# ADicksonLab/AGDIFF

Hardware: AMD Instinct MI355X
Metric: conformers/sec (whole node), GEOM-Drugs 5000-step sampling (higher is better)
Workload: dtype f16x3

## Files before the change

agdiff_amd/csrc/api.hip:

```cpp
#include "common.hpp"
#include <algorithm>
#include <mutex>
#include <vector>

extern "C" int agdiff_abi_version(void) { return AGDIFF_ABI_VERSION; }

extern "C" int agdiff_conv_chunk_tiles(int64_t max_edges) {
  const int64_t tiles = (max_edges + AG_TW - 1) / AG_TW;
  int c = 1;
  while (c < AGDIFF_MAX_CHUNK_TILES && tiles / (2 * c) >= 16 * 2048) c *= 2;
  return c;
}

extern "C" int agdiff_group_order(const int32_t* need, int32_t n, int32_t k, int32_t gt, int32_t* order_out) {
  if (n < 0 || k < 0 || (gt != 1 && gt != 2 && gt != 4) || (n > 0 && (!need || !order_out))) return AGDIFF_ERR_ARG;
  if (n == 0) return AGDIFF_OK;
  auto row = [&](int i) { return need + (size_t)i * k; };
  std::vector<int> total(n, 0);
  for (int i = 0; i < n; ++i)
    for (int t = 0; t < k; ++t) total[i] += row(i)[t];
  auto start_order = [&](int r, std::vector<int>& o) {
    o.resize(n);
    for (int i = 0; i < n; ++i) o[i] = i;
    std::stable_sort(o.begin(), o.end(), [&](int a, int b) {
// ... 157 lines not shown
  }
  return f;
}

int local_branch(const agdiff_params_t* p, const agdiff_topo_t* topo, const agdiff_ws_t* ws, const float* pos, int flags,
                 bool rows_from_global, hipEvent_t rows_ready, void* stream, bool split = false,
                 hipEvent_t split_ready = nullptr) {
  const int64_t ltiles = (topo->num_local + AG_TW - 1) / AG_TW;
  const int64_t ctiles = (topo->num_local_canon + AG_TW - 1) / AG_TW;
  const bool canon = !(flags & AGDIFF_FWD_GRAPH_GIVEN) && topo->num_local_canon > 0;
  const bool front_did_local = (flags & AGDIFF_FWD_GRAPH_READY) != 0;
  if (!(flags & AGDIFF_FWD_GRAPH_GIVEN) && !front_did_local) AG_TRY(agdiff_local_lengths(topo, ws, pos, stream));
  if (rows_from_global) {
    if (hipStreamWaitEvent((hipStream_t)stream, rows_ready, 0) != hipSuccess) return AGDIFF_ERR_LAUNCH;
  } else if (topo->num_local > 0) {
    if (canon && split) {
      const int lp = agdiff_local_poly_enabled(p, topo, ws);
      if (lp != 0 && !front_did_local) AG_TRY(agdiff_edge_scales_split(p, topo, ws, 2, stream));
      if (lp == 1) {
        AG_TRY(agdiff_local_edge_rows(p, topo, ws, stream));
      } else {
        AG_TRY(agdiff_edge_encoder(p, ws->num_local_canon, ctiles, ws->lc_len, topo->lc_type, ws->l_attr_frag, ws->l_attr_rows,
                                   topo->lp_row, topo->lc_ppos, topo->lc_pmir, stream));
        AG_TRY(agdiff_edge_scales_split(p, topo, ws, 1, stream));
      }
    } else if (canon)
      AG_TRY(agdiff_local_edge_rows(p, topo, ws, stream));
    else
      AG_TRY(agdiff_edge_encoder(p, ws->num_local, ltiles, ws->l_len, topo->loc_type, nullptr, ws->l_attr_rows, nullptr,
                                 nullptr, nullptr, stream));
  }
  if (split && split_ready && hipEventRecord(split_ready, (hipStream_t)stream) != hipSuccess) return AGDIFF_ERR_LAUNCH;
  AG_TRY(agdiff_gin_encoder(p, topo, ws, canon ? 1 : 0, stream));
  if (topo->num_local > 0) {
    agdiff_head_params_t hl = p->head_local;
    hl.range_rows = ws->range_rows;
    if (canon)
      AG_TRY(agdiff_pair_head(&hl, ws->num_local_canon, ctiles, topo->lc_src, topo->lc_dst, ws->hl, nullptr,
                              ws->l_attr_rows, topo->lc_pos, topo->lc_mir, ws->l_inv, stream));
    else
      AG_TRY(agdiff_pair_head(&hl, ws->num_local, ltiles, topo->loc_src, topo->loc_dst, ws->hl, nullptr,
                              ws->l_attr_rows, nullptr, nullptr, ws->l_inv, stream));
  }
  return AGDIFF_OK;
}

int global_front(const agdiff_params_t* p, const agdiff_topo_t* topo, const agdiff_ws_t* ws, const float* pos, int flags,
                 bool rows_for_local, void* stream) {
  const int64_t etiles = (topo->max_edges + AG_TW - 1) / AG_TW;
  if (!(flags & AGDIFF_FWD_GRAPH_GIVEN))
    AG_TRY(agdiff_graph_build(topo, ws, pos, (flags & AGDIFF_FWD_NO_RADIUS) ? 0.0f : p->cutoff, stream));
  AG_TRY(agdiff_edge_scales(p, topo, ws, (flags & AGDIFF_FWD_GRAPH_GIVEN) ? 0 : 1, stream));
  if (flags & AGDIFF_FWD_GRAPH_GIVEN) {
    AG_TRY(agdiff_edge_encoder(p, ws->num_edges, etiles, ws->e_len, ws->e_type, ws->e_attr, nullptr, nullptr, nullptr,
                               nullptr, stream));
  } else {
    AG_TRY(agdiff_edge_encoder(p, ws->num_canon, etiles, ws->c_len, ws->c_type, ws->e_attr,
                               rows_for_local ? ws->l_attr_rows : nullptr, rows_for_local ? ws->e_loc : nullptr, ws->c_pos,
                               ws->c_mir, stream));
  }
  return AGDIFF_OK;
}

int global_back(const agdiff_params_t* p, const agdiff_topo_t* topo, const agdiff_ws_t* ws, int flags, void* stream) {
  const int64_t etiles = (topo->max_edges + AG_TW - 1) / AG_TW;
  for (int k = 0; k <= p->num_convs; ++k) {
    AG_TRY(agdiff_schnet_node_stage(p, topo, ws, k, stream));
    if (k < p->num_convs) {
      ProfScope prof(stream);
      AG_TRY(agdiff_cfconv_fused(p, topo, ws, k, stream));
    }
  }
  agdiff_head_params_t hg = p->head_global;
  hg.range_rows = ws->range_rows;
  if (flags & AGDIFF_FWD_GRAPH_GIVEN) {
    AG_TRY(agdiff_pair_head(&hg, ws->num_edges, etiles, ws->e_src, ws->e_dst, ws->h, ws->e_attr, nullptr,
// ... 164 lines not shown
```

agdiff_amd/csrc/edge.hip:

```cpp
#include "common.hpp"

namespace {

__device__ __forceinline__ const lds_u32x4* ag_lds_base(const lds_u32x4* p, int lane) {
  const lds_u32x4* b = p + lane;
  asm volatile("" : "+v"(b));
  return b;
}

struct EncArgs {
  const float* fe_w;
  const float* fe_b;
  const float* t1;
  const float* w1_pk;
  const float* t3;
  const float* w23_pk;
  const float* w4_pk;
  const float* b4;
  const int32_t* n_dev;
  const float* e_len;
  const int32_t* e_type;
  float* out_frag;
  float* out_rows;
  const int32_t* row_index;
// ... 787 lines not shown
        ag_load_slice_pieces(r[0], r[1], hs, k, lane);
        ag_load_slice_pieces(r[2], r[3], ht, k, lane);
      };
      auto finish = [&](AgIn<MODE>& dst, const f32x4 (&r)[4]) {
        ag_cvt(ag_permute4(r[0] * r[2], to_op), ag_permute4(r[1] * r[3], to_op), dst);
      };
      fetch(raw, 0);
      finish(sl[0], raw);
      const lds_u32x4* lw1_l = ag_lds_base(lw1, lane);
#pragma unroll
      for (int k = 0; k < 4; ++k) {
        if (k + 1 < 4) fetch(raw, k + 1);
        if (k & 1) ag_dense_lds<MODE, false, true, 1, 8, 1, 0>(sl, y1, lw1_l + (k * 8) * 128, 0);
        else ag_dense_lds<MODE, false, true, 1, 8, 0, 0>(sl, y1, lw1_l + (k * 8) * 128, 0);
        if (k + 1 < 4) finish(sl[(k + 1) & 1], raw);
      }
      AgIn<MODE> ph[NKT];
      ag_poly_features<MODE, NKT>(d, a.two_over_rc, q, ph);
      ag_dense_lds<MODE, false, true, NKT, 8, 0, 0>(ph, y1, ag_lds_base(lwp, lane), 0);
    }
    ag_head_act<8>(y1, a.hp.act);
    f32x4 y2[4];
    ag_init_vec<4>(y2, a.hp.b2, q);
    {
      AgIn<MODE> y1b[4];
      ag_report_range<MODE>(ag_absmax<MODE, 8>(y1, 0.0f), a.hp.range_rows, s, valid);
      ag_cvt_tiles<MODE, 4, 0>(y1, y1b);
      ag_dense_lds<MODE, false, false, 4, 4, 0, 0>(y1b, y2, ag_lds_base(lw2, lane), 0);
    }
    ag_head_act<4>(y2, a.hp.act);
    const float o = ag_dot_vec<4>(y2, a.hp.w3, q) + a.hp.b3;
    if (valid && q == 0) {
      a.out[pe] = o;
      if (pm >= 0) a.out[pm] = o;
    }
  }
}

template <int F>
__global__ void __launch_bounds__(AG_WG) k_cfconv_aggregate(const float* __restrict__ x, const float* __restrict__ W,
                                                            const int32_t* __restrict__ in_ptr,
                                                            const int32_t* __restrict__ src, int64_t n,
                                                            float* __restrict__ out) {
  constexpr int LPE = F / 4;
  constexpr int EPI = 64 / LPE;
  const int lane = ag_lane();
  const int64_t node = (int64_t)blockIdx.x * 4 + ag_wave_in_wg();
  if (node >= n) return;
  const int lo = in_ptr[node], hi = in_ptr[node + 1];
  const int sub = lane / LPE, fl = (lane % LPE) * 4;
  f32x4 acc = {0.f, 0.f, 0.f, 0.f};
  for (int e = lo + sub; e < hi; e += EPI) {
    const f32x4 w = ag_ld4(W + (size_t)e * F + fl);
    const f32x4 xv = ag_ld4(x + (size_t)src[e] * F + fl);
    acc += w * xv;
  }
#pragma unroll
  for (int o = LPE; o < 64; o <<= 1) {
#pragma unroll
    for (int q = 0; q < 4; ++q) acc[q] += __shfl_xor(acc[q], o);
  }
  if (sub == 0) ag_st4(out + (size_t)node * F + fl, acc);
}

}

// ... 300 lines not shown

extern "C" int agdiff_pair_head(const agdiff_head_params_t* hp, const int32_t* n_edges_dev, int64_t max_tiles,
                                const int32_t* src, const int32_t* dst, const float* node_h, const float* attr_frag,
                                const float* attr_rows, const int32_t* pos_index, const int32_t* mir_index, float* out,
                                void* stream) {
  if (!hp || !n_edges_dev || !src || !dst || !node_h || (!attr_frag == !attr_rows) || !out || max_tiles < 0 ||
      (!pos_index != !mir_index))
    return AGDIFF_ERR_ARG;
  if (max_tiles == 0) return AGDIFF_OK;
  HeadArgs a;
  a.hp = *hp;
  a.n_dev = n_edges_dev;
  a.src = src;
  a.dst = dst;
  a.node_h = node_h;
  a.attr_frag = attr_frag;
  a.attr_rows = attr_rows;
  a.pos_index = pos_index;
  a.mir_index = mir_index;
  a.out = out;
  a.max_tiles = max_tiles;
  int64_t wgs = (max_tiles + AG_PERSIST_WAVES - 1) / AG_PERSIST_WAVES;
  if (wgs > 256) wgs = 256;
  const size_t smem = (size_t)80 * 2048;
  static std::atomic<uint64_t> attr_done{0};
  if (!ag_allow_big_lds(attr_done, smem, k_pair_head<AG_BF3>, k_pair_head<AG_F32>, k_pair_head<AG_H3>)) return AGDIFF_ERR_LAUNCH;
  ag_by_mode(hp->precision, [&](auto M) {
    k_pair_head<decltype(M)::value><<<dim3((unsigned)wgs), dim3(64 * AG_PERSIST_WAVES), smem, (hipStream_t)stream>>>(a);
  });
  AG_CHECK_LAUNCH();
  return AGDIFF_OK;
}

extern "C" int agdiff_cfconv_aggregate(const float* x, const float* W, const int32_t* in_ptr, const int32_t* src,
                                       int64_t num_nodes, int32_t F, float* out, void* stream) {
  if (!x || !W || !in_ptr || !src || !out || num_nodes < 0) return AGDIFF_ERR_ARG;
  if (F != 64 && F != 128) return AGDIFF_ERR_LIMIT;
  if (num_nodes == 0) return AGDIFF_OK;
  dim3 grid((unsigned)((num_nodes + 3) / 4));
  if (F == 128)
    k_cfconv_aggregate<128><<<grid, dim3(AG_WG), 0, (hipStream_t)stream>>>(x, W, in_ptr, src, num_nodes, out);
  else
    k_cfconv_aggregate<64><<<grid, dim3(AG_WG), 0, (hipStream_t)stream>>>(x, W, in_ptr, src, num_nodes, out);
  AG_CHECK_LAUNCH();
  return AGDIFF_OK;
}
```

agdiff_amd/packing.py:

```python
import ctypes

import numpy as np

from . import _lib

H = 128


def _np(sd, key):
    return sd[key].detach().cpu().double().numpy()


def bf16_round(x32):
    u = np.ascontiguousarray(x32, dtype=np.float32).view(np.uint32).astype(np.uint64)
    r = ((u + 0x7FFF + ((u >> 16) & 1)) >> 16).astype(np.uint32)
    return r.astype(np.uint16), (r << 16).astype(np.uint32).view(np.float32)


def _block_columns():
    lane = np.arange(64)
    j = np.arange(8)
    return 16 * (j >> 2)[None, :] + 4 * (lane >> 4)[:, None] + (j & 3)[None, :]


# ... 112 lines not shown
    G.append(2 * T8 * T8 - 1)
    G.append(2 * G[2] * T8 - T8)
    G.append(2 * G[2] * G[2] - 1)
    G.append(2 * G[4] * T8 - G[3])
    G.append(2 * G[3] * G[3] - 1)
    G.append(2 * G[6] * T8 - G[5])
    while len(G) < K // 8:
        G.append(2 * T8 * G[-1] - G[-2])
    return np.stack([G[f // 8] * T[f % 8] for f in range(K)], axis=-1)


def fit_poly(fn, cutoff, K, lo=0.0):
    k = np.arange(K)
    xn = np.cos(np.pi * (k + 0.5) / K)
    half = (cutoff - lo) / 2.0
    fv = fn(lo + (xn + 1.0) * half)
    b = np.polynomial.chebyshev.chebfit(xn, fv, K - 1)
    c = np.linalg.solve(poly_basis_matrix(K), b)
    dg = np.linspace(lo, cutoff, 4097)
    ref = fn(dg)
    err = np.abs(poly_features((dg - lo) / half - 1.0, K) @ c - ref).max() / max(np.abs(ref).max(), 1e-300)
    return c.T, float(err)


ATTR_FAR_FACTOR = 10.0
ATTR_POLY_MAX_SETS = 9


def fit_attr_far(sd, cfg, typ):
    key = (_poly_weights_digest(sd, cfg), float(cfg.cutoff), int(typ), "attr_far")
    if key not in _FIT_CACHE:
        fn = _edge_attr_fn(sd, "edge_encoder_global", typ)
        c, err = fit_poly(lambda d: fn(d).numpy(), ATTR_FAR_FACTOR * float(cfg.cutoff), 32, lo=float(cfg.cutoff))
        _FIT_CACHE[key] = (c[:, poly_feature_order(1)], err)
    return _FIT_CACHE[key]


def _edge_attr_fn(sd, e, typ):
    import torch
    import torch.nn.functional as F
    g = lambda k: sd[e + k].detach().cpu().double()
    few, feb = g(".feature_expansion.weight"), g(".feature_expansion.bias")
    W0, b0, W2, b2 = g(".edge_feature_mlp.0.weight"), g(".edge_feature_mlp.0.bias"), g(".edge_feature_mlp.2.weight"), g(".edge_feature_mlp.2.bias")
    C0, c0, C2, c2 = g(".combination_mlp.0.weight"), g(".combination_mlp.0.bias"), g(".combination_mlp.2.weight"), g(".combination_mlp.2.bias")
    emb = g(".bond_emb.weight")[int(typ)]

    def fn(d):
        d = torch.from_numpy(np.ascontiguousarray(d, dtype=np.float64)).view(-1, 1)
        x = F.gelu(F.linear(d, few, feb))
        b = emb.expand(d.shape[0], -1)
        h = F.linear(F.gelu(F.linear(torch.cat([x, b], 1), W0, b0)), W2, b2)
        return F.linear(F.gelu(F.linear(torch.cat([h, b], 1), C0, c0)), C2, c2)
    return fn


def encoder_activation_by_type(sd, cfg, far=10.0):
    import torch
    import torch.nn.functional as F
    e = "edge_encoder_global"
    g = lambda k: sd[k].detach().cpu().double()
    few, feb = g(e + ".feature_expansion.weight"), g(e + ".feature_expansion.bias")
    W0, b0, W2, b2 = g(e + ".edge_feature_mlp.0.weight"), g(e + ".edge_feature_mlp.0.bias"), g(e + ".edge_feature_mlp.2.weight"), g(e + ".edge_feature_mlp.2.bias")
    C0, c0, C2, c2 = g(e + ".combination_mlp.0.weight"), g(e + ".combination_mlp.0.bias"), g(e + ".combination_mlp.2.weight"), g(e + ".combination_mlp.2.bias")
    emb = g(e + ".bond_emb.weight")
    d = torch.linspace(0.0, float(far) * float(cfg.cutoff), 1025, dtype=torch.float64).view(-1, 1)
    x = F.gelu(F.linear(d, few, feb))
# ... 531 lines not shown
            self.poly_errors["type%d" % t] = err
            if err > POLY_TOL or len(self.local_slots) >= max_slots or not self._type_fits_plan(t, mats, err):
                self.poly_refused_types.add(t)
                continue
            self.local_slots[t] = len(self.local_slots)
            self._typed_mats[t] = mats
            added = True
        if not added:
            return not any(int(t) in self.poly_refused_types for t in types)
        by_slot = sorted(self.local_slots, key=self.local_slots.get)
        self._pack_filter_sets()
        if kt == 1:
            sets = [pack_blocks(self._typed_mats[t]["edge_attr_poly_pk"], mode=self._mode_local) for t in by_slot]
            far_table = np.full(100, -1, dtype=np.int32)
            room = max(0, ATTR_POLY_MAX_SETS - len(by_slot)) if self.attr_far else 0
            prio = {24: 0, 23: 1, 1: 2}
            for t in sorted(by_slot, key=lambda ty: (prio.get(ty, 3), ty)):
                if room <= 0:
                    break
                c, err = fit_attr_far(self._sd, self._cfg, t)
                self.poly_errors["type%d_far" % t] = err
                if err > POLY_TOL:
                    continue
                far_table[t] = len(sets)
                sets.append(pack_blocks(c, mode=self._mode_local))
                room -= 1
            attr_sets = np.concatenate(sets)
            self.typed_attr_flat = torch.from_numpy(attr_sets).to(self.device)
            prm.attr_poly_typed_pk = ctypes.c_void_p(self.typed_attr_flat.data_ptr())
            self.attr_far_table = torch.from_numpy(far_table).to(self.device)
            prm.attr_poly_far_set = ctypes.c_void_p(self.attr_far_table.data_ptr())
            prm.attr_poly_far_slots = int((far_table >= 0).sum())
            prm.attr_poly_far_hi = ATTR_FAR_FACTOR * float(self._cfg.cutoff)
        table = np.full(100, -1, dtype=np.int32)
        for t, sl in self.local_slots.items():
            table[t] = sl
        self.slot_table = torch.from_numpy(table).to(self.device)
        prm.poly_type_slot = ctypes.c_void_p(self.slot_table.data_ptr())
        prm.poly_num_slots = len(by_slot)
        sm = [0, 0]
        for t in self.local_slots:
            sm[t >> 6] |= 1 << (t & 63)
        for w in (0, 1):
            prm.poly_slot_mask[w] = sm[w] - (1 << 64) if sm[w] >= (1 << 63) else sm[w]
        return not any(int(t) in self.poly_refused_types for t in types)

    TUNING = ("share_rows_min_nodes", "node_ldsw_min_tiles", "node_split_max_tiles", "serial_branches", "local_poly_off",
              "attr_poly_off", "poly_lds_sets", "cfconv_four_min_quads", "cfconv_quad_tiles")

    def set_tuning(self, **kw):
        for k, v in kw.items():
            if k not in self.TUNING:
                raise KeyError("unknown tuning field %r (known: %s)" % (k, ", ".join(self.TUNING)))
            setattr(self.struct, "tune_" + k, int(v))

    def view(self, name):
        o = self.offsets[name]
        return self.flat[o:o + self.sizes[name]]

    def update_schnet_embedding(self, weight):
        self.view("schnet_emb").copy_(weight.detach().reshape(-1).to(self.flat.dtype))
```

agdiff_amd/topology.py:

```python
import numpy as np

from . import _lib
from .synth import extend_graph_order_np


def _to_np(x):
    if hasattr(x, "detach"):
        x = x.detach().cpu().numpy()
    return np.asarray(x)


def batch_fingerprint(atom_type, bond_index, bond_type, batch, num_graphs, extend_order):
    def wsum(cols, mults):
        if hasattr(cols[0], "detach"):
            import torch
            n = int(cols[0].reshape(-1).shape[0])
            if n == 0:
                return 0
            acc = torch.zeros(n, dtype=torch.int64, device=cols[0].device)
            for c, m in zip(cols, mults):
                acc += c.reshape(-1).to(torch.int64) * m
            acc = (acc + 12345) * torch.arange(1, n + 1, dtype=torch.int64, device=acc.device)
            return int(acc.sum().item())
        cols = [np.asarray(c).reshape(-1).astype(np.int64) for c in cols]
# ... 33 lines not shown

def extend_graph_order_sparse(n, bond_src, bond_dst, bond_type, order=3, num_types=None):
    from .synth import NUM_BOND_TYPES
    num_types = NUM_BOND_TYPES if num_types is None else num_types
    n = int(n)
    bs, bd = np.asarray(bond_src, dtype=np.int64), np.asarray(bond_dst, dtype=np.int64)
    bkey, inv = np.unique(bs * n + bd, return_inverse=True)
    tsum = np.zeros(bkey.shape[0], dtype=np.int64)
    np.add.at(tsum, inv.reshape(-1), np.asarray(bond_type, dtype=np.int64))
    offdiag = (bkey // n) != (bkey % n)
    adj = bkey[offdiag]
    a_src, a_dst = adj // n, adj % n
    nb_ptr = np.concatenate([[0], np.cumsum(np.bincount(a_src, minlength=n))])
    seen = np.union1d(np.arange(n, dtype=np.int64) * (n + 1), adj)
    frontier = adj
    keys, types = [bkey], [tsum]
    for k in range(2, order + 1):
        f_src, f_dst = frontier // n, frontier % n
        deg = nb_ptr[f_dst + 1] - nb_ptr[f_dst]
        rep_src = np.repeat(f_src, deg)
        first = np.repeat(nb_ptr[f_dst], deg)
        within = np.arange(rep_src.shape[0]) - np.repeat(np.cumsum(deg) - deg, deg)
        cand = np.unique(rep_src * n + a_dst[first + within])
        frontier = np.setdiff1d(cand, seen, assume_unique=True)
        seen = np.union1d(seen, frontier)
        keys.append(frontier)
        types.append(np.full(frontier.shape[0], num_types + k - 1, dtype=np.int64))
    key = np.concatenate(keys)
    typ = np.concatenate(types)
    o = np.argsort(key, kind="stable")
    key, typ = key[o], typ[o]
    keep = typ != 0
    return key[keep] // n, key[keep] % n, typ[keep]


class BatchTopology:
    GROUP_MIN_NODES = ((6144, 4), (3072, 2))

    def __init__(self, atom_type, bond_index, bond_type, batch, num_graphs=None, extend_order=False,
                 order=3, device="cuda", group_targets=None, radius_column=True):
        import torch
        at = _to_np(atom_type).astype(np.int64)
        bi = _to_np(bond_index).astype(np.int64).reshape(2, -1)
        bt = _to_np(bond_type).astype(np.int64).reshape(-1)
        ba = _to_np(batch).astype(np.int64)
        self.fingerprint = batch_fingerprint(at, bi, bt, ba, num_graphs, extend_order)
        N = at.shape[0]
        if ba.shape[0] != N:
            raise ValueError("batch and atom_type disagree on the number of nodes")
        if N == 0:
            raise ValueError("empty batch")
        if np.any(np.diff(ba) < 0):
            raise ValueError("batch must be sorted (graph-contiguous nodes, PyG Batch.from_data_list)")
        G = int(ba[-1]) + 1 if num_graphs is None else int(num_graphs)
        counts = np.bincount(ba, minlength=G)
        gptr = np.concatenate([[0], np.cumsum(counts)]).astype(np.int64)
        if at.min() < 0 or at.max() >= 100:
            raise ValueError("atom_type out of the embedding range [0, 100)")
        if bi.size and (bi.min() < 0 or bi.max() >= N):
            raise ValueError("bond_index out of range")
        if bi.size and np.any(ba[bi[0]] != ba[bi[1]]):
            raise ValueError("bond between different graphs")

        if extend_order:
            rs, cs, ts = [], [], []
            order_src = np.argsort(ba[bi[0]], kind="stable") if bi.size else np.zeros(0, dtype=np.int64)
# ... 159 lines not shown
        if L:
            k_of = np.searchsorted(ltypes, typ)
            tile_e = tile_of_qk[quad_of[dst] * qneed.shape[1] + k_of] + rank_in // RT
            tpos = tile_e * 16 + slot_of[dst] * RT + rank_in % RT
        real_t = np.zeros(16 * T, dtype=bool)
        eid_t = np.full(16 * T, -1, dtype=np.int64)
        real_t[tpos] = True
        eid_t[tpos] = np.arange(L)
        assert int(real_t.sum()) == L
        trow = np.arange(16 * T)
        tgt_t = qt[tile_quad[trow // 16], (trow % 16) // RT] if T else np.zeros(0, dtype=np.int64)
        first_t = qt[tile_quad[trow // 16], 0] if T else tgt_t
        tgt_c = np.where(tgt_t >= 0, tgt_t, first_t)
        self.T, self.Q, self.group_targets = T, int(Q), GT
        self.quad_tgt = i32(quad_tgt)
        self.lt_ptr = i32(lt_ptr)
        self.lt_src = i32(np.where(real_t, src[np.maximum(eid_t, 0)], tgt_c) if L else np.zeros(16 * T))
        self.lt_type = i32(ltypes[tile_type_k][trow // 16] if T else np.zeros(0))
        self.lt_real = real_t
        self.quad_wg_ptr = i32(wg_ptr) if wg_ptr.size else None
        if self.large:
            self.loc_bits = None
        else:
            W = 2 * ((self.max_atoms + 63) // 64)
            bits = np.zeros(N * W, dtype=np.uint32)
            if L:
                jl = src - gptr[ba[src]]
                bits = np.bincount(dst * W + (jl >> 5), weights=np.ldexp(1.0, (jl & 31).astype(np.int32)), minlength=N * W).astype(np.uint32)
            self.loc_bits = torch.from_numpy(bits.view(np.int32)).to(device)
        self.lt_eid = eid_t
        self.lc_tpos = i32(tpos[lc_pos])
        self.lc_tmir = i32(np.where(lc_mir >= 0, tpos[np.maximum(lc_mir, 0)], -1))
        self.lcm_ptr = i32(np.searchsorted(ba[src[lc_pos]], np.arange(G + 1)) if L else np.zeros(G + 1))
        self.local_types = np.unique(typ)
        self.loc_index64 = torch.from_numpy(np.stack([src, dst])).to(device)
        self.loc_type64 = torch.from_numpy(typ).to(device)
        self.batch64 = torch.from_numpy(ba).to(device)
        self.graph_sizes = counts

        t = _lib.Topo()
        t.num_nodes, t.num_graphs, t.num_local = N, G, L
        t.max_edges, t.max_atoms_per_graph, t.max_in_degree = self.max_edges, self.max_atoms, self.max_in_degree
        t.num_local_canon = self.Lc
        t.num_local_padded = self.Lp
        t.num_local_tiles = self.T
        t.num_quads = self.Q
        t.group_targets = self.group_targets
        tm = [0, 0]
        for ty in self.local_types:
            tm[int(ty) >> 6] |= 1 << (int(ty) & 63)
        for w in (0, 1):
            t.local_type_mask[w] = tm[w] - (1 << 64) if tm[w] >= (1 << 63) else tm[w]
        self.struct = t
        self._set_pointers()

    _POINTER_FIELDS = ("graph_ptr", "atom_type", "loc_src", "loc_dst", "loc_type", "loc_out_ptr", "loc_in_ptr", "loc_in_eid",
                       "lc_src", "lc_dst", "lc_type", "lc_pos", "lc_mir", "loc_row", "loc_in_src",
                       "loc_in_row", "lp_ptr", "lp_src", "lp_dst", "lp_type", "lp_row", "lc_ppos", "lc_pmir",
                       "quad_tgt", "lt_ptr", "lt_src", "lt_type", "lc_tpos", "lc_tmir", "lcm_ptr", "loc_bits")

    def _set_pointers(self):
        for f in self._POINTER_FIELDS:
            setattr(self.struct, f, _lib.ptr(getattr(self, f)))
        self.struct.quad_wg_ptr = _lib.ptr(self.quad_wg_ptr) if self.quad_wg_ptr is not None else None

    def __getstate__(self):
        import ctypes
        st = dict(self.__dict__)
        t = st.pop("struct")
        scalars = {}
        for name, ctype in _lib.Topo._fields_:
            if ctype is ctypes.c_void_p:
                continue
            v = getattr(t, name)
            scalars[name] = list(v) if hasattr(v, "__len__") else v
        st["_struct_scalars"] = scalars
        return st

    def __setstate__(self, st):
        scalars = st.pop("_struct_scalars")
        self.__dict__.update(st)
        t = _lib.Topo()
        for name, v in scalars.items():
            if isinstance(v, list):
                for k, x in enumerate(v):
                    getattr(t, name)[k] = x
            else:
                setattr(t, name, v)
        self.struct = t
        self._set_pointers()

    def to(self, device):
# ... 87 lines not shown
```

include/agdiff_hip.h:

```cpp
#ifndef AGDIFF_HIP_H
#define AGDIFF_HIP_H

#include <stdint.h>

#ifdef __cplusplus
extern "C" {
#endif

#define AGDIFF_ABI_VERSION 48
#define AGDIFF_HIDDEN 128
#define AGDIFF_MAX_CONVS 8
#define AGDIFF_MAX_CONVS_LOCAL 8
#define AGDIFF_NUM_EDGE_TYPES 100
#define AGDIFF_MAX_ATOMS_PER_GRAPH 512
#define AGDIFF_MAX_ATOMS_LARGE 16384
#define AGDIFF_RADIUS_CAP 33
#define AGDIFF_TILE 16
#define AGDIFF_MAX_CHUNK_TILES 8
#define AGDIFF_RMSD_MAX_ATOMS 256
#define AGDIFF_PRUNE_MAX_CONFS 4096
#define AGDIFF_KMEDOIDS_MAX_DIST 4096
#define AGDIFF_KMEDOIDS_MAX_ITER 128
#define AGDIFF_KMEDOIDS_WORK_BYTES 131072
#define AGDIFF_SILHOUETTE_WORK_BYTES 65536
// ... 104 lines not shown
  const int32_t* poly_type_slot;
  const float* dist_union;
  const float* attr_poly_typed_pk;
  agdiff_conv_params_t conv[AGDIFF_MAX_CONVS];
  agdiff_gin_params_t gin[AGDIFF_MAX_CONVS_LOCAL];
  agdiff_head_params_t head_global;
  agdiff_head_params_t head_local;
  int32_t num_convs;
  int32_t num_convs_local;
  float cutoff;
  int32_t smooth;
  int32_t precision;
  int32_t edge_encoder;
  float ge_coeff;
  int32_t poly_num_slots;
  int32_t precision_local;
  int32_t poly_kt;
  int32_t poly_plan;
  int32_t tune_cfconv_quad_tiles;
  int64_t poly_slot_mask[2];
  int64_t tune_share_rows_min_nodes;
  int64_t tune_node_ldsw_min_tiles;
  int64_t tune_node_split_max_tiles;
  int32_t tune_serial_branches;
  int32_t tune_local_poly_off;
  int32_t tune_attr_poly_off;
  int32_t tune_poly_lds_sets;
  int32_t attr_poly_far_slots;
  const int32_t* attr_poly_far_set;
  float attr_poly_far_hi;
  int64_t tune_cfconv_four_min_quads;
  int32_t dist_union_kinks;
  int32_t dist_union_segments;
} agdiff_params_t;

#define AGDIFF_VAR_CFCONV_NODE 1
#define AGDIFF_VAR_CFCONV_NODE_LOCAL 2
#define AGDIFF_VAR_CFCONV_LOCAL_MLP 4
#define AGDIFF_VAR_CFCONV_FUSED 8
#define AGDIFF_VAR_NODE_LDSW 16
#define AGDIFF_VAR_NODE_STREAM 32
#define AGDIFF_VAR_NODE_SPLIT4 64
#define AGDIFF_VAR_GIN_LDSW 128
#define AGDIFF_VAR_SHARE_ROWS 256
#define AGDIFF_VAR_ATTR_POLY 512
#define AGDIFF_VAR_HEAD_POLY 1024
#define AGDIFF_VAR_SIDE_STREAM 2048
#define AGDIFF_VAR_POLY_L2_SETS 4096
#define AGDIFF_VAR_FUSED_FRONT 8192
#define AGDIFF_VAR_CFCONV_NODE_FOUR 16384
#define AGDIFF_VAR_CFCONV_NODE_QUAD 32768
#define AGDIFF_VAR_GRAPH_LARGE 65536

typedef struct agdiff_topo {
  int64_t num_nodes;
  int64_t num_graphs;
  int64_t num_local;
  int64_t max_edges;
  int64_t max_atoms_per_graph;
  int64_t max_in_degree;
  const int32_t* graph_ptr;
  const int32_t* atom_type;
  const int32_t* loc_src;
  const int32_t* loc_dst;
  const int32_t* loc_type;
  const int32_t* loc_out_ptr;
  const int32_t* loc_in_ptr;
  const int32_t* loc_in_eid;
  int64_t num_local_canon;
  const int32_t* lc_src;
  const int32_t* lc_dst;
  const int32_t* lc_type;
  const int32_t* lc_pos;
  const int32_t* lc_mir;
  const int32_t* loc_row;
  const int32_t* loc_in_src;
  const int32_t* loc_in_row;
  int64_t num_local_padded;
  const int32_t* lp_ptr;
  const int32_t* lp_src;
  const int32_t* lp_dst;
  const int32_t* lp_type;
  const int32_t* lp_row;
  const int32_t* lc_ppos;
  const int32_t* lc_pmir;
  int64_t num_quads;
  int64_t group_targets;
  const int32_t* quad_tgt;
  const int32_t* lcm_ptr;
  int64_t local_type_mask[2];
  int64_t num_local_tiles;
  const int32_t* lt_ptr;
  const int32_t* lt_src;
  const int32_t* lt_type;
  const int32_t* lc_tpos;
  const int32_t* lc_tmir;
  const int32_t* quad_wg_ptr;
  const int32_t* loc_bits;
} agdiff_topo_t;

typedef struct agdiff_ws {
  int32_t* num_edges;
  int32_t* num_local;
  int32_t* graph_edge_cnt;
  int32_t* graph_edge_ptr;
  int32_t* in_ptr;
  int32_t* out_ptr;
  int32_t* e_src;
  int32_t* e_dst;
  int32_t* e_type;
  float*   e_len;
  int32_t* ref2dst;
  int32_t* e_loc;
  int32_t* num_canon;
  int32_t* graph_canon_cnt;
  int32_t* graph_canon_ptr;
  float*   c_len;
  int32_t* c_type;
  int32_t* c_src;
  int32_t* c_dst;
  int32_t* c_pos;
  int32_t* c_mir;
  float*   e_attr;
  float*   e_inv_global;
  float*   e_scale;
  float*   l_len;
  float*   lc_len;
  int32_t* num_local_canon;
  float*   l_attr_rows;
  float*   l_inv;
// ... 93 lines not shown
                     const int32_t* src, const int32_t* dst, const float* node_h, const float* attr_frag,
                     const float* attr_rows, const int32_t* pos_index, const int32_t* mir_index, float* out,
                     void* stream);

int agdiff_gin_encoder(const agdiff_params_t* p, const agdiff_topo_t* topo, const agdiff_ws_t* ws,
                       int32_t rows_per_canonical_edge, void* stream);

int agdiff_cfconv_aggregate(const float* x, const float* W, const int32_t* in_ptr, const int32_t* src,
                            int64_t num_nodes, int32_t F, float* out, void* stream);

#define AGDIFF_FWD_GLOBAL 1
#define AGDIFF_FWD_NO_RADIUS 2
#define AGDIFF_FWD_GRAPH_GIVEN 4
#define AGDIFF_FWD_SAMPLER 8
#define AGDIFF_FWD_STAGE0_CACHED 16
#define AGDIFF_FWD_GRAPH_READY 32
#define AGDIFF_FWD_PARITY 64
#define AGDIFF_FWD_GRAPH_PENDING 128
int agdiff_score_forward(const agdiff_params_t* p, const agdiff_topo_t* topo, const agdiff_ws_t* ws,
                         const float* pos, int32_t flags, void* stream);

int agdiff_sampler_front(const agdiff_params_t* p, const agdiff_topo_t* topo, const agdiff_ws_t* ws,
                         const agdiff_step_args_t* s, int32_t mode, float cutoff, void* stream);
int agdiff_step_graph_capture(const agdiff_params_t* p, const agdiff_topo_t* topo, const agdiff_ws_t* ws,
                              const agdiff_step_args_t* host_step , const agdiff_step_args_t* step_table,
                              int32_t* step_index, int32_t front_mode, float cutoff, int32_t fwd_flags, void* stream,
                              void** graph_out );
int agdiff_step_graph_launch(void* graph , void* stream);
int agdiff_step_graph_destroy(void* graph );

int agdiff_pair_head_poly_rows(const agdiff_params_t* p, const agdiff_topo_t* topo, const agdiff_ws_t* ws, int32_t parity,
                               void* stream);

int agdiff_profile_cfconv(int32_t enable);
int agdiff_profile_cfconv_read(double* total_ms, int64_t* launches);

int agdiff_langevin_update(const agdiff_topo_t* topo, const agdiff_ws_t* ws, const agdiff_step_args_t* a, void* stream);

int agdiff_counter_noise(const agdiff_topo_t* topo, const int64_t* stream_id , uint64_t seed,
                         const int32_t* steps , int32_t num_steps,
                         float* out , void* stream);

int agdiff_perturb_positions(const agdiff_topo_t* topo, const float* pos, const float* noise,
                             const float* alpha_graph, float* pos_out, void* stream);

int agdiff_diffusion_loss(const agdiff_params_t* p, const agdiff_topo_t* topo, const agdiff_ws_t* ws,
                          const float* pos_gt, const float* pos_perturbed, const float* alpha_graph,
                          float* loss, void* stream);

int agdiff_langevin_step(const agdiff_params_t* p, const agdiff_topo_t* topo, const agdiff_ws_t* ws,
                         const agdiff_step_args_t* a, void* stream);

int agdiff_rmsd_matrix(const float* pos_ref, const float* pos_gen, const int32_t* atom_idx, const int32_t* perms,
                       int32_t R, int32_t G, int32_t n, int32_t m, int32_t P, float* scratch, float* out, void* stream);

int agdiff_matrix_minima(const float* mat, int32_t R, int32_t G, float* row_min, float* col_min, void* stream);

int agdiff_rmsd_self(const float* pos, const int32_t* atom_idx, const int32_t* perms, int32_t G, int32_t n, int32_t m,
                     int32_t P, float thresh, float* scratch, float* out, uint64_t* bits, void* stream);

int agdiff_leader_prune(const uint64_t* bits, int32_t G, int32_t* keep, int32_t* leader, int32_t* count, int32_t* n_kept,
                        void* stream);

int agdiff_butina_cluster(const uint64_t* bits, int32_t G, int32_t reorder, int32_t* leader, int32_t* count, int32_t* rank,
                          int32_t* n_clusters, void* stream);

// ... 110 lines not shown
```

Before: 177.8.

## Add typed local pair-head kernel using per-type polynomial fits of attr projection

Adds a new local pair-head kernel that sorts canonical local edges into type-homogeneous 16-edge tiles. When every edge in a tile falls inside the near (or far) distance band, the kernel replaces the edge-attribute half of the first dense layer with a precomputed per-type polynomial in distance, with coefficients held in LDS. Mixed tiles fall back to loading attribute rows from memory. This avoids reading attr rows and four K-blocks of matmul per tile, at the cost of padding tiles (up to about 8%), extra topology arrays, and polynomial approximation error bounded by a tolerance check.

```diff
diff --git a/agdiff_amd/csrc/api.hip b/agdiff_amd/csrc/api.hip
--- a/agdiff_amd/csrc/api.hip
+++ b/agdiff_amd/csrc/api.hip
@@ -213,16 +213,7 @@
   }
   if (split && split_ready && hipEventRecord(split_ready, (hipStream_t)stream) != hipSuccess) return AGDIFF_ERR_LAUNCH;
   AG_TRY(agdiff_gin_encoder(p, topo, ws, canon ? 1 : 0, stream));
-  if (topo->num_local > 0) {
-    agdiff_head_params_t hl = p->head_local;
-    hl.range_rows = ws->range_rows;
-    if (canon)
-      AG_TRY(agdiff_pair_head(&hl, ws->num_local_canon, ctiles, topo->lc_src, topo->lc_dst, ws->hl, nullptr,
-                              ws->l_attr_rows, topo->lc_pos, topo->lc_mir, ws->l_inv, stream));
-    else
-      AG_TRY(agdiff_pair_head(&hl, ws->num_local, ltiles, topo->loc_src, topo->loc_dst, ws->hl, nullptr,
-                              ws->l_attr_rows, nullptr, nullptr, ws->l_inv, stream));
-  }
+  if (topo->num_local > 0) AG_TRY(agdiff_local_head(p, topo, ws, canon ? 1 : 0, stream));
   return AGDIFF_OK;
 }
 
diff --git a/agdiff_amd/csrc/edge.hip b/agdiff_amd/csrc/edge.hip
--- a/agdiff_amd/csrc/edge.hip
+++ b/agdiff_amd/csrc/edge.hip
@@ -843,6 +843,127 @@
     const float o = ag_dot_vec<4>(y2, a.hp.w3, q) + a.hp.b3;
     if (valid && q == 0) {
       a.out[pe] = o;
+      if (pm >= 0) a.out[pm] = o;
+    }
+  }
+}
+
+struct HeadTypedArgs {
+  agdiff_head_params_t hp;
+  const int32_t* idx;
+  const int32_t* src;
+  const int32_t* dst;
+  const int32_t* pos;
+  const int32_t* mir;
+  const int32_t* tile_type;
+  const float* len;
+  const float* node_h;
+  const float* attr_rows;
+  const float* sets;
+  const int32_t* near_set;
+  const int32_t* far_set;
+  float* out;
+  int64_t tiles;
+  int32_t lds_sets;
+  float cutoff;
+  float two_over_rc;
+  float far_hi;
+  float two_over_far;
+};
+#define AG_HEADT_LDS_SETS 4
+
+template <int MODE>
+__global__ void __launch_bounds__(64 * AG_PERSIST_WAVES, 4) k_pair_head_typed(HeadTypedArgs a) {
+  extern __shared__ u32x4 ag_headt_smem[];
+  lds_u32x4* lw1 = (lds_u32x4*)ag_headt_smem;
+  lds_u32x4* lw2 = lw1 + 32 * 128;
+  lds_u32x4* lws = lw2 + 16 * 128;
+  ag_copy_lds(lw1, reinterpret_cast<const u32x4*>(a.hp.w1_pk), 32 * 128);
+  ag_copy_lds(lw2, reinterpret_cast<const u32x4*>(a.hp.w2_pk), 16 * 128);
+  if (a.lds_sets > 0) ag_copy_lds(lws, reinterpret_cast<const u32x4*>(a.sets), a.lds_sets * 8 * 128);
+  __syncthreads();
+  const int lane0 = ag_lane();
+  const int64_t stride = (int64_t)gridDim.x * AG_PERSIST_WAVES;
+  const int64_t wg = (gridDim.x % 8 == 0) ? (int64_t)(blockIdx.x % 8) * (gridDim.x / 8) + blockIdx.x / 8 : (int64_t)blockIdx.x;
+  for (int64_t tile = wg * AG_PERSIST_WAVES + (threadIdx.x >> 6); tile < a.tiles; tile += stride) {
+    int lane = lane0;
+    asm volatile("" : "+v"(lane));
+    const int q = lane >> 4;
+    const int64_t e = tile * AG_TW + (lane & 15);
+    const int c = a.idx[e];
+    const bool valid = c >= 0;
+    const int s = valid ? a.src[e] : 0, t = valid ? a.dst[e] : 0;
+    const float d = valid ? a.len[c] : 0.0f;
+    const int ty = a.tile_type[tile];
+    const int nset = a.near_set[ty], fset = a.far_set ? a.far_set[ty] : -1;
+    const bool is_nan = (__float_as_uint(d) & 0x7FFFFFFFu) > 0x7F800000u;
+    const bool in_near = !is_nan && d >= 0.0f && d <= a.cutoff;
+    const bool in_far = !is_nan && d > a.cutoff && d <= a.far_hi;
+    const bool all_near = nset >= 0 && __ballot(valid && !in_near) == 0;
+    const bool all_far = !all_near && fset >= 0 && __ballot(valid && !in_far) == 0;
+    const int set = all_near ? nset : all_far ? fset : -1;
+
+    f32x4 y1[8];
+    ag_init_vec<8>(y1, a.hp.b1, q);
+    {
+      const float* hs = a.node_h + (size_t)ag_piece_row_value(s, lane) * 128;
+      const float* ht = a.node_h + (size_t)ag_piece_row_value(t, lane) * 128;
+      const int to_op = ag_to_operand_addr(lane);
+      AgIn<MODE> sl[2];
+      f32x4 raw[4];
+      auto fetch = [&](f32x4 (&r)[4], int k) {
+        ag_load_slice_pieces(r[0], r[1], hs, k, lane);
+        ag_load_slice_pieces(r[2], r[3], ht, k, lane);
+      };
+      auto finish = [&](AgIn<MODE>& dst, const f32x4 (&r)[4]) {
+        ag_cvt(ag_permute4(r[0] * r[2], to_op), ag_permute4(r[1] * r[3], to_op), dst);
+      };
+      fetch(raw, 0);
+      finish(sl[0], raw);
+      const lds_u32x4* lw1_l = ag_lds_base(lw1, lane);
+#pragma unroll
+      for (int k = 0; k < 4; ++k) {
+        if (k + 1 < 4) fetch(raw, k + 1);
+        if (k & 1) ag_dense_lds<MODE, false, true, 1, 8, 1, 0>(sl, y1, lw1_l + (k * 8) * 128, 0);
+        else ag_dense_lds<MODE, false, true, 1, 8, 0, 0>(sl, y1, lw1_l + (k * 8) * 128, 0);
+        if (k + 1 < 4) finish(sl[(k + 1) & 1], raw);
+      }
+      if (set >= 0) {
+        AgIn<MODE> ph[1];
+        ag_poly_features<MODE, 1>(all_near ? d : d - a.cutoff, all_near ? a.two_over_rc : a.two_over_far, q, ph);
+        if (set < a.lds_sets)
+          ag_dense_lds<MODE, false, true, 1, 8, 0, 0>(ph, y1, ag_lds_base(lws + (size_t)set * (8 * 128), lane), 0);
+        else
+          ag_dense<MODE, false, true, 1, 8, 0, 0, 2>(ph, y1, a.sets + (size_t)set * (8 * 512), lane);
+      } else {
+        const float* ar = a.attr_rows + (size_t)ag_piece_row_value(valid ? c : 0, lane) * 128;
+#pragma unroll 1
+        for (int k = 0; k < 4; ++k) {
+          f32x4 r0, r1;
+          ag_load_slice_pieces(r0, r1, ar, k, lane);
+          AgIn<MODE> x[1];
+          ag_cvt(ag_permute4(r0, to_op), ag_permute4(r1, to_op), x[0]);
+          ag_dense<MODE, false, true, 1, 8, 0, 0, 2>(x, y1, ag_wblock(a.hp.w1_pk, (4 + k) * 8), lane);
+        }
+      }
+    }
+    ag_head_act<8>(y1, a.hp.act);
+    f32x4 y2[4];
+    ag_init_vec<4>(y2, a.hp.b2, q);
+    {
+      AgIn<MODE> y1b[4];
+      ag_report_range<MODE>(ag_absmax<MODE, 8>(y1, 0.0f), a.hp.range_rows, s, valid);
+      ag_cvt_tiles<MODE, 4, 0>(y1, y1b);
+      ag_dense_lds<MODE, false, false, 4, 4, 0, 0>(y1b, y2, ag_lds_base(lw2, lane), 0);
+    }
+    ag_head_act<4>(y2, a.hp.act);
+    const float o = ag_dot_vec<4>(y2, a.hp.w3, q) + a.hp.b3;
+    if (valid && q == 0) {
+      int l2 = lane0;
+      asm volatile("" : "+v"(l2));
+      const int64_t e2 = tile * AG_TW + (l2 & 15);
+      a.out[a.pos[e2]] = o;
+      const int pm = a.mir[e2];
       if (pm >= 0) a.out[pm] = o;
     }
   }
@@ -1209,6 +1330,62 @@
   return AGDIFF_OK;
 }
 
+extern "C" int agdiff_local_head(const agdiff_params_t* p, const agdiff_topo_t* topo, const agdiff_ws_t* ws, int32_t canonical,
+                                 void* stream) {
+  if (!p || !topo || !ws || !ws->hl || !ws->l_attr_rows || !ws->l_inv) return AGDIFF_ERR_ARG;
+  if (topo->num_local == 0) return AGDIFF_OK;
+  agdiff_head_params_t hl = p->head_local;
+  hl.range_rows = ws->range_rows;
+  if (!canonical)
+    return agdiff_pair_head(&hl, ws->num_local, (topo->num_local + AG_TW - 1) / AG_TW, topo->loc_src, topo->loc_dst, ws->hl, nullptr,
+                            ws->l_attr_rows, nullptr, nullptr, ws->l_inv, stream);
+  const bool typed = !p->tune_local_head_poly_off && p->edge_encoder == 0 && p->poly_kt == 1 && p->head_local_poly_pk &&
+                     p->head_local_near_set && p->head_local_near_sets > 0 && topo->num_head_tiles > 0 && topo->lh_idx &&
+                     topo->lh_src && topo->lh_dst && topo->lh_pos && topo->lh_mir && topo->lh_type && ws->lc_len;
+  if (!typed)
+    return agdiff_pair_head(&hl, ws->num_local_canon, (topo->num_local_canon + AG_TW - 1) / AG_TW, topo->lc_src, topo->lc_dst, ws->hl,
+                            nullptr, ws->l_attr_rows, topo->lc_pos, topo->lc_mir, ws->l_inv, stream);
+  if (p->head_local_far_sets < 0 || (p->head_local_far_sets > 0 && (!p->head_local_far_set || !(p->attr_poly_far_hi > p->cutoff))))
+    return AGDIFF_ERR_ARG;
+  HeadTypedArgs a;
+  a.hp = hl;
+  a.idx = topo->lh_idx;
+  a.src = topo->lh_src;
+  a.dst = topo->lh_dst;
+  a.pos = topo->lh_pos;
+  a.mir = topo->lh_mir;
+  a.tile_type = topo->lh_type;
+  a.len = ws->lc_len;
+  a.node_h = ws->hl;
+  a.attr_rows = ws->l_attr_rows;
+  a.sets = p->head_local_poly_pk;
+  a.near_set = p->head_local_near_set;
+  a.far_set = p->head_local_far_sets > 0 ? p->head_local_far_set : nullptr;
+  a.out = ws->l_inv;
+  a.tiles = topo->num_head_tiles;
+  const int nsets = p->head_local_near_sets + p->head_local_far_sets;
+  int lds = p->tune_local_head_lds_sets < 0 ? 0 : (int)ag_tune(p->tune_local_head_lds_sets, AG_HEADT_LDS_SETS);
+  if (lds > AG_HEADT_LDS_SETS) lds = AG_HEADT_LDS_SETS;
+  a.lds_sets = lds < nsets ? lds : nsets;
+  a.cutoff = p->cutoff;
+  a.two_over_rc = 2.0f / p->cutoff;
+  a.far_hi = a.far_set ? p->attr_poly_far_hi : p->cutoff;
+  a.two_over_far = a.far_set ? 2.0f / (p->attr_poly_far_hi - p->cutoff) : 0.0f;
+  int64_t wgs = (a.tiles + AG_PERSIST_WAVES - 1) / AG_PERSIST_WAVES;
+  if (wgs > 256) wgs = 256;
+  const size_t smem = (size_t)(48 + 8 * a.lds_sets) * 2048;
+  static std::atomic<uint64_t> attr_done{0};
+  if (!ag_allow_big_lds(attr_done, (size_t)(48 + 8 * AG_HEADT_LDS_SETS) * 2048, k_pair_head_typed<AG_BF3>, k_pair_head_typed<AG_F32>,
+                        k_pair_head_typed<AG_H3>))
+    return AGDIFF_ERR_LAUNCH;
+  ag_by_mode(hl.precision, [&](auto M) {
+    k_pair_head_typed<decltype(M)::value><<<dim3((unsigned)wgs), dim3(64 * AG_PERSIST_WAVES), smem, (hipStream_t)stream>>>(a);
+  });
+  AG_CHECK_LAUNCH();
+  ag_log_variant(ws, AGDIFF_VAR_LOCAL_HEAD_POLY);
+  return AGDIFF_OK;
+}
+
 extern "C" int agdiff_cfconv_aggregate(const float* x, const float* W, const int32_t* in_ptr, const int32_t* src,
                                        int64_t num_nodes, int32_t F, float* out, void* stream) {
   if (!x || !W || !in_ptr || !src || !out || num_nodes < 0) return AGDIFF_ERR_ARG;
diff --git a/agdiff_amd/packing.py b/agdiff_amd/packing.py
--- a/agdiff_amd/packing.py
+++ b/agdiff_amd/packing.py
@@ -168,6 +168,20 @@
     if key not in _FIT_CACHE:
         fn = _edge_attr_fn(sd, "edge_encoder_global", typ)
         c, err = fit_poly(lambda d: fn(d).numpy(), ATTR_FAR_FACTOR * float(cfg.cutoff), 32, lo=float(cfg.cutoff))
+        _FIT_CACHE[key] = (c[:, poly_feature_order(1)], err)
+    return _FIT_CACHE[key]
+
+
+def fit_head_local(sd, cfg, typ, far=False):
+    Wb = sd["grad_local_dist_mlp.layers.0.weight"].detach().cpu().double()[:, H:]
+    import hashlib
+    key = (_poly_weights_digest(sd, cfg), hashlib.sha1(np.ascontiguousarray(Wb.numpy()).tobytes()).hexdigest(), float(cfg.cutoff),
+           int(typ), bool(far), "head_local")
+    if key not in _FIT_CACHE:
+        attr = _edge_attr_fn(sd, "edge_encoder_global", typ)
+        fn = lambda d: (attr(d) @ Wb.T).numpy()
+        rc = float(cfg.cutoff)
+        c, err = fit_poly(fn, ATTR_FAR_FACTOR * rc, 32, lo=rc) if far else fit_poly(fn, rc, 32)
         _FIT_CACHE[key] = (c[:, poly_feature_order(1)], err)
     return _FIT_CACHE[key]
 
@@ -765,6 +779,7 @@
             prm.attr_poly_far_set = ctypes.c_void_p(self.attr_far_table.data_ptr())
             prm.attr_poly_far_slots = int((far_table >= 0).sum())
             prm.attr_poly_far_hi = ATTR_FAR_FACTOR * float(self._cfg.cutoff)
+            self._pack_local_head_sets(by_slot)
         table = np.full(100, -1, dtype=np.int32)
         for t, sl in self.local_slots.items():
             table[t] = sl
@@ -778,8 +793,38 @@
             prm.poly_slot_mask[w] = sm[w] - (1 << 64) if sm[w] >= (1 << 63) else sm[w]
         return not any(int(t) in self.poly_refused_types for t in types)
 
+    def _pack_local_head_sets(self, by_slot):
+        import torch
+        prm = self.struct
+        n0 = self.head_norm["head_local"][0]
+        near, far = np.full(100, -1, dtype=np.int32), np.full(100, -1, dtype=np.int32)
+        sets = []
+        for want_far, table in ((False, near), (True, far)):
+            if want_far and not self.attr_far:
+                break
+            for t in by_slot:
+                c, err = fit_head_local(self._sd, self._cfg, t, far=want_far)
+                self.poly_errors["head_local_type%d%s" % (t, "_far" if want_far else "")] = err
+                if err > POLY_TOL or (want_far and near[t] < 0):
+                    continue
+                table[t] = len(sets)
+                sets.append(pack_blocks(np.asarray(c, dtype=np.float64) * n0, kouter=True, mode=self._mode_local))
+        self.head_local_sets = {"near": near, "far": far}
+        if not sets:
+            prm.head_local_poly_pk = prm.head_local_near_set = prm.head_local_far_set = None
+            prm.head_local_near_sets = prm.head_local_far_sets = 0
+            return
+        self.head_local_flat = torch.from_numpy(np.concatenate(sets)).to(self.device)
+        self.head_local_tables = torch.from_numpy(np.concatenate([near, far])).to(self.device)
+        prm.head_local_poly_pk = ctypes.c_void_p(self.head_local_flat.data_ptr())
+        prm.head_local_near_set = ctypes.c_void_p(self.head_local_tables.data_ptr())
+        prm.head_local_far_set = ctypes.c_void_p(self.head_local_tables.data_ptr() + 400)
+        prm.head_local_near_sets = int((near >= 0).sum())
+        prm.head_local_far_sets = int((far >= 0).sum())
+
     TUNING = ("share_rows_min_nodes", "node_ldsw_min_tiles", "node_split_max_tiles", "serial_branches", "local_poly_off",
-              "attr_poly_off", "poly_lds_sets", "cfconv_four_min_quads", "cfconv_quad_tiles")
+              "attr_poly_off", "poly_lds_sets", "cfconv_four_min_quads", "cfconv_quad_tiles", "local_head_poly_off",
+              "local_head_lds_sets")
 
     def set_tuning(self, **kw):
         for k, v in kw.items():
diff --git a/agdiff_amd/topology.py b/agdiff_amd/topology.py
--- a/agdiff_amd/topology.py
+++ b/agdiff_amd/topology.py
@@ -89,6 +89,32 @@
     key, typ = key[o], typ[o]
     keep = typ != 0
     return key[keep] // n, key[keep] % n, typ[keep]
+
+
+HEAD_TILE_MAX_PAD = 0.08
+
+
+def head_tile_permutation(mol, typ, max_pad=HEAD_TILE_MAX_PAD):
+    mol, typ = np.asarray(mol, dtype=np.int64), np.asarray(typ, dtype=np.int64)
+    n = mol.shape[0]
+    if n == 0:
+        return np.zeros(0, dtype=np.int64), np.zeros(0, dtype=np.int64), 1
+    assert np.all(np.diff(mol) >= 0) and typ.min() >= 0 and typ.max() < 128
+    R, n_mol = 1, int(mol[-1]) + 1
+    while True:
+        key = (mol // R) * 128 + typ
+        order = np.argsort(key, kind="stable")
+        seg_key, seg_first, seg_cnt = np.unique(key[order], return_index=True, return_counts=True)
+        padded = (seg_cnt + 15) // 16 * 16
+        total = int(padded.sum())
+        if total - n <= max_pad * total or R >= n_mol:
+            break
+        R *= 2
+    seg_of = np.repeat(np.arange(seg_key.shape[0]), seg_cnt)
+    pos = (np.cumsum(padded) - padded)[seg_of] + np.arange(n) - seg_first[seg_of]
+    idx = np.full(total, -1, dtype=np.int64)
+    idx[pos] = order
+    return idx, np.repeat(seg_key % 128, padded // 16), R
 
 
 class BatchTopology:
@@ -314,6 +340,12 @@
         self.lc_tpos = i32(tpos[lc_pos])
         self.lc_tmir = i32(np.where(lc_mir >= 0, tpos[np.maximum(lc_mir, 0)], -1))
         self.lcm_ptr = i32(np.searchsorted(ba[src[lc_pos]], np.arange(G + 1)) if L else np.zeros(G + 1))
+        lh_idx, lh_type, self.head_run_molecules = head_tile_permutation(ba[src[lc_pos]], typ[lc_pos])
+        lh_real, lh_c = lh_idx >= 0, np.maximum(lh_idx, 0)
+        self.Th = int(lh_type.shape[0])
+        self.lh_idx, self.lh_type = i32(lh_idx), i32(lh_type)
+        self.lh_src, self.lh_dst = i32(np.where(lh_real, src[lc_pos][lh_c], 0) if L else lh_idx), i32(np.where(lh_real, dst[lc_pos][lh_c], 0) if L else lh_idx)
+        self.lh_pos, self.lh_mir = i32(np.where(lh_real, lc_pos[lh_c], -1) if L else lh_idx), i32(np.where(lh_real, lc_mir[lh_c], -1) if L else lh_idx)
         self.local_types = np.unique(typ)
         self.loc_index64 = torch.from_numpy(np.stack([src, dst])).to(device)
         self.loc_type64 = torch.from_numpy(typ).to(device)
@@ -326,6 +358,7 @@
         t.num_local_canon = self.Lc
         t.num_local_padded = self.Lp
         t.num_local_tiles = self.T
+        t.num_head_tiles = self.Th
         t.num_quads = self.Q
         t.group_targets = self.group_targets
         tm = [0, 0]
@@ -339,7 +372,8 @@
     _POINTER_FIELDS = ("graph_ptr", "atom_type", "loc_src", "loc_dst", "loc_type", "loc_out_ptr", "loc_in_ptr", "loc_in_eid",
                        "lc_src", "lc_dst", "lc_type", "lc_pos", "lc_mir", "loc_row", "loc_in_src",
                        "loc_in_row", "lp_ptr", "lp_src", "lp_dst", "lp_type", "lp_row", "lc_ppos", "lc_pmir",
-                       "quad_tgt", "lt_ptr", "lt_src", "lt_type", "lc_tpos", "lc_tmir", "lcm_ptr", "loc_bits")
+                       "quad_tgt", "lt_ptr", "lt_src", "lt_type", "lc_tpos", "lc_tmir", "lcm_ptr", "loc_bits",
+                       "lh_idx", "lh_src", "lh_dst", "lh_pos", "lh_mir", "lh_type")
 
     def _set_pointers(self):
         for f in self._POINTER_FIELDS:
diff --git a/include/agdiff_hip.h b/include/agdiff_hip.h
--- a/include/agdiff_hip.h
+++ b/include/agdiff_hip.h
@@ -160,6 +160,13 @@
   int64_t tune_cfconv_four_min_quads;
   int32_t dist_union_kinks;
   int32_t dist_union_segments;
+  const float* head_local_poly_pk;
+  const int32_t* head_local_near_set;
+  const int32_t* head_local_far_set;
+  int32_t head_local_near_sets;
+  int32_t head_local_far_sets;
+  int32_t tune_local_head_poly_off;
+  int32_t tune_local_head_lds_sets;
 } agdiff_params_t;
 
 #define AGDIFF_VAR_CFCONV_NODE 1
@@ -178,6 +185,7 @@
 #define AGDIFF_VAR_FUSED_FRONT 8192
 #define AGDIFF_VAR_CFCONV_NODE_FOUR 16384
 #define AGDIFF_VAR_CFCONV_NODE_QUAD 32768
+#define AGDIFF_VAR_LOCAL_HEAD_POLY 131072
 #define AGDIFF_VAR_GRAPH_LARGE 65536
 
 typedef struct agdiff_topo {
@@ -224,6 +232,13 @@
   const int32_t* lc_tpos;
   const int32_t* lc_tmir;
   const int32_t* quad_wg_ptr;
+  int64_t num_head_tiles;
+  const int32_t* lh_idx;
+  const int32_t* lh_src;
+  const int32_t* lh_dst;
+  const int32_t* lh_pos;
+  const int32_t* lh_mir;
+  const int32_t* lh_type;
   const int32_t* loc_bits;
 } agdiff_topo_t;
 
@@ -383,6 +398,8 @@
 int agdiff_pair_head_poly_rows(const agdiff_params_t* p, const agdiff_topo_t* topo, const agdiff_ws_t* ws, int32_t parity,
                                void* stream);
 
+int agdiff_local_head(const agdiff_params_t* p, const agdiff_topo_t* topo, const agdiff_ws_t* ws, int32_t canonical, void* stream);
+
 int agdiff_profile_cfconv(int32_t enable);
 int agdiff_profile_cfconv_read(double* total_ms, int64_t* launches);
 
```

Result: faster. 179.9 (median of 6 runs) (+1.2%).
